# gssales/gaussian-splatting-reflection

Measured on AMD Instinct MI355X. Metric: train_step_views_per_s (fwd+bwd, 1e6 Gaussians @1080p, surfel rasterizer + reflection path), higher is better.
Workload: dtype f32

## Files before the change

### gaussian-splatting-reflection_amd/_gsr.py

```python
import ctypes
import os

import torch

_HERE = os.path.dirname(os.path.abspath(__file__))
LIB_PATH = os.environ.get("GSR_LIB") or os.path.join(_HERE, "libgsr_hip.so")

c_void_p, c_int, c_float, c_size_t, c_uint32, c_char_p = (ctypes.c_void_p, ctypes.c_int, ctypes.c_float, ctypes.c_size_t,
                                                         ctypes.c_uint32, ctypes.c_char_p)
ALLOC_FN = ctypes.CFUNCTYPE(c_void_p, c_void_p, c_int, c_size_t)

GSR_BUF_GEOM, GSR_BUF_BINNING, GSR_BUF_IMAGE = 0, 1, 2
GSR_PRESENT_CLAMP, GSR_PRESENT_QUANT8 = 1, 2
GSR_VIEW_HALF, GSR_VIEW_SOBEL, GSR_VIEW_COLORMAP = 1, 2, 4


class GsrError(RuntimeError):
    pass


class GatherGroup(ctypes.Structure):
    _fields_ = [("src_offset", ctypes.c_uint64), ("dst_offset", ctypes.c_uint64), ("width", c_uint32)]


# ... 136 lines not shown
def compiled_binding():
    want = os.environ.get("GSR_BINDING", "auto")
    if want == "ctypes":
        return None
    import importlib.util
    path = os.path.join(_HERE, "_gsr_C.so")
    if not os.path.exists(path):
        if want == "pybind":
            raise ImportError(f"GSR_BINDING=pybind but {path} is not built: run `python {os.path.join(_HERE, 'csrc', 'build.py')} --binding`")
        return None
    try:
        spec = importlib.util.spec_from_file_location("_gsr_C", path)
        mod = importlib.util.module_from_spec(spec)
        spec.loader.exec_module(mod)
        return mod
    except Exception:
        if want == "pybind":
            raise
        return None


PYBIND = compiled_binding()

EXPORTED = ["gsr_last_error", "gsr_version", "gsr_surfel_forward", "gsr_surfel_backward", "gsr_surfel_backward_accum", "gsr_surfel_backward_ex",
            "gsr_surfel_forward_refl", "gsr_surfel_forward_eval", "gsr_deferred_reflection_backward_keys", "gsr_deferred_reflection_forward_keys",
            "gsr_deferred_reflection_backward_accum", "gsr_deferred_reflection_backward_ex", "gsr_deferred_reflection_forward_ex", "gsr_side_join", "gsr_normal_world_forward", "gsr_normal_world_backward", "gsr_gauss_forward", "gsr_gauss_backward", "gsr_gauss_backward_accum",
            "gsr_mark_visible", "gsr_debug_fetch", "gsr_cubemap_forward", "gsr_cubemap_backward", "gsr_deferred_reflection_forward",
            "gsr_deferred_reflection_scratch_floats", "gsr_deferred_reflection_backward", "gsr_ssim_l1_scratch_floats", "gsr_ssim_l1_forward", "gsr_ssim_l1_backward", "gsr_normal_loss_scratch_floats", "gsr_normal_loss_forward", "gsr_normal_loss_backward", "gsr_adam_step", "gsr_adam_step_range", "gsr_densification_stats", "gsr_gather_rows", "gsr_split_children", "gsr_surface_forward", "gsr_surface_backward", "gsr_profile_enable",
            "gsr_profile_collect", "gsr_set_option", "gsr_knn_scratch_bytes", "gsr_knn_mean_dist",
            "gsr_image_metrics_scratch_floats", "gsr_image_metrics", "gsr_normal_mae_scratch_floats", "gsr_normal_mae",
            "gsr_present_view_scratch_floats", "gsr_present_view"]

STAGES = ["preprocess", "scan_readback", "emit_keys", "sort", "tile_ranges", "render_fwd", "render_bwd", "preprocess_bwd", "refl_fwd",
          "refl_bwd", "cubemap_fwd", "cubemap_bwd", "loss_fwd", "loss_bwd", "adam", "surface_fwd", "surface_bwd", "refl_bwd_tail"]


def set_option(name, value):
    check(lib.gsr_set_option(name.encode(), int(value)), f"gsr_set_option({name})")


_side_held = {}


def side_hold(*tensors):
    for t in tensors:
        if t is None:
            continue
        dev = t.device.index if t.device.index is not None else torch.cuda.current_device()
        _side_held.setdefault(dev, []).append((t, torch.cuda.current_stream(t.device).cuda_stream))


def side_join(device=None):
    dev = torch.device("cuda", torch.cuda.current_device()) if device is None else torch.device(device)
    if dev.index is None:
        dev = torch.device("cuda", torch.cuda.current_device())
    held = _side_held.pop(dev.index, [])
    with torch.cuda.device(dev):
        cur = torch.cuda.current_stream(dev).cuda_stream
        check(lib.gsr_side_join(cur), "gsr_side_join")
        for s in {s for _, s in held if s != cur}:
            check(lib.gsr_side_join(s), "gsr_side_join")
    del held


def profile_enable(on=True):
    lib.gsr_profile_enable(1 if on else 0)

# ... 107 lines not shown
```

### gaussian-splatting-reflection_amd/csrc/gsr_common.hip

```cpp
#include "gsr_internal.hpp"
#include <cstdarg>
#include <string>
#include <initializer_list>
#include <vector>
#include <mutex>
#include "gsr_sort.hpp"
#include <rocprim/device/device_scan.hpp>
#include <rocprim/iterator/counting_iterator.hpp>
#include <rocprim/iterator/transform_iterator.hpp>

namespace gsr {

static thread_local char g_err[512] = "";
void set_error(const char* fmt, ...) {
	va_list ap;
	va_start(ap, fmt);
	vsnprintf(g_err, sizeof(g_err), fmt, ap);
	va_end(ap);
}


struct ProfRec {
	int stage;
	hipEvent_t e0, e1;
// ... 5 lines not shown

StageTimer::StageTimer(int stage_, hipStream_t stream_) : stage(stage_), stream(stream_), rec(nullptr) {
	if (!g_prof_on) return;
	std::lock_guard<std::mutex> lk(g_prof_mu);
	ProfRec* r = nullptr;
	if (!g_prof_free.empty()) {
		r = g_prof_free.back();
		g_prof_free.pop_back();
	} else {
		r = new ProfRec();
		if (hipEventCreate(&r->e0) != hipSuccess || hipEventCreate(&r->e1) != hipSuccess) { delete r; return; }
	}
	r->stage = stage;
	(void)hipEventRecord(r->e0, stream);
	rec = r;
}
StageTimer::~StageTimer() {
	if (!rec) return;
	ProfRec* r = (ProfRec*)rec;
	(void)hipEventRecord(r->e1, stream);
	std::lock_guard<std::mutex> lk(g_prof_mu);
	g_prof_recs.push_back(r);
}

static int g_opt_cull = 1;
int option_cull() { return g_opt_cull; }
static int g_opt_dev = 0;
int option_dev() { return g_opt_dev; }
static int g_opt_emit_items = 0;
static int g_opt_mailbox = 1;
static int option_mailbox() { return g_opt_mailbox; }
static int g_opt_sort_driver = GSR_ONESWEEP_DRIVER;
int option_sort_driver() { return GSR_ONESWEEP_DRIVER && g_opt_sort_driver; }

uint32_t higher_msb(uint32_t n) {
	uint32_t msb = sizeof(n) * 4;
	uint32_t step = msb;
	while (step > 1) {
		step /= 2;
		if (n >> msb) msb += step;
		else msb -= step;
	}
	if (n >> msb) msb++;
	return msb;
}

using SortConfig = rocprim::radix_sort_config<rocprim::default_config, rocprim::default_config, rocprim::default_config, 65536>;
#ifndef DEPTH_SORT_BS
#define DEPTH_SORT_BS 1024
#endif
#ifndef DEPTH_SORT_IPT
#define DEPTH_SORT_IPT 4
#endif
#define DEPTH_SORT_SHAPE DEPTH_SORT_BS, DEPTH_SORT_IPT, 8
#define DEPTH_KEY_BITS 31u
#define DEPTH_KEY_PLACES 4u
#ifndef TILE_SORT_IPT
#define TILE_SORT_IPT 16
#endif
#ifndef TILE_SORT_BITS
#define TILE_SORT_BITS 8
#endif
#ifndef TILE_SORT_BS
#define TILE_SORT_BS 1024
#endif
#define TILE_SORT_SHAPE TILE_SORT_BS, TILE_SORT_IPT, TILE_SORT_BITS
// ... 506 lines not shown
	out[3 * idx + 0] = b & 1;
	out[3 * idx + 1] = (b >> 1) & 1;
	out[3 * idx + 2] = (b >> 2) & 1;
}
struct RecPick { int n; int pos[9]; };
__global__ void __launch_bounds__(256) pick_rec_kernel(int P, const float* __restrict__ rec, int stride, RecPick pick, float* __restrict__ out) {
	const int i = blockIdx.x * 256 + threadIdx.x;
	if (i >= P * pick.n) return;
	const int idx = i / pick.n, k = i % pick.n;
	out[i] = rec[(size_t)idx * stride + pick.pos[k]];
}
__global__ void __launch_bounds__(256) gather_rec_kernel(int P, const float* __restrict__ rec, int stride, int first, int nf,
                                                         float* __restrict__ out) {
	const int i = blockIdx.x * 256 + threadIdx.x;
	if (i >= P * nf) return;
	const int idx = i / nf, k = i % nf;
	out[i] = rec[(size_t)idx * stride + first + k];
}

}

using namespace gsr;

extern "C" const char* gsr_last_error(void) { return g_err; }
extern "C" int gsr_version(void) { return GSR_ABI_VERSION; }


extern "C" int gsr_set_option(const char* name, int value) {
	if (std::string(name) == "cull") { g_opt_cull = value ? 1 : 0; return 0; }
	if (std::string(name) == "dev") { g_opt_dev = value; return 0; }
	if (std::string(name) == "emit_items") { g_opt_emit_items = (value == 1 || value == 2) ? value : 0; return 0; }
	if (std::string(name) == "mailbox") { g_opt_mailbox = value ? 1 : 0; return 0; }
	if (std::string(name) == "sort_driver") { g_opt_sort_driver = value ? 1 : 0; return 0; }
	set_error("gsr_set_option: unknown option '%s'", name);
	return GSR_E_INVALID;
}
extern "C" int gsr_profile_enable(int on) {
	std::lock_guard<std::mutex> lk(g_prof_mu);
	for (ProfRec* r : g_prof_recs) g_prof_free.push_back(r);
	g_prof_recs.clear();
	g_prof_on = on != 0;
	return 0;
}
extern "C" int gsr_profile_collect(float* ms_out, int* launches_out) {
	std::lock_guard<std::mutex> lk(g_prof_mu);
	for (int i = 0; i < GSR_STAGE_COUNT; i++) { if (ms_out) ms_out[i] = 0.f; if (launches_out) launches_out[i] = 0; }
	for (ProfRec* r : g_prof_recs) {
		float ms = 0.f;
		if (hipEventSynchronize(r->e1) == hipSuccess && hipEventElapsedTime(&ms, r->e0, r->e1) == hipSuccess) {
			if (ms_out) ms_out[r->stage] += ms;
			if (launches_out) launches_out[r->stage] += 1;
		}
		g_prof_free.push_back(r);
	}
	g_prof_recs.clear();
	return 0;
}

extern "C" int gsr_mark_visible(int P, const float* means3D, const float* viewmatrix, const float* projmatrix, uint8_t* present,
                                void* stream_) {
	(void)projmatrix;
	hipStream_t stream = (hipStream_t)stream_;
	if (P < 0 || (P > 0 && (!means3D || !viewmatrix || !present))) { set_error("gsr_mark_visible: invalid argument"); return GSR_E_INVALID; }
	if (P == 0) return 0;
	mark_visible_kernel<<<(P + 255) / 256, 256, 0, stream>>>(P, means3D, viewmatrix, present);
	GSR_LAUNCH_CHECK(0, stream);
	return 0;
}

extern "C" int gsr_debug_fetch(int variant, const char* name, int P, int R, int width, int height, const void* geom_buffer,
                               const void* binning_buffer, const void* image_buffer, void* dst, void* stream_) {
	hipStream_t stream = (hipStream_t)stream_;
	const int tiles_x = (width + 15) / 16, tiles_y = (height + 15) / 16;
	const size_t HW = (size_t)width * height, tiles = (size_t)tiles_x * tiles_y;
	const WorkspaceLayout& layout = variant == 0 ? SURFEL_LAYOUT : GAUSS_LAYOUT;
	const int stride = layout.rec_f4 * 4;
	GeomState g = carve_geom((void*)geom_buffer, P, layout, nullptr);
	ImageState im = carve_image((void*)image_buffer, HW, tiles, layout, nullptr);
	BinningState b = carve_binning((void*)binning_buffer, R, tiles, 0, nullptr);
	auto d2d = [&](const void* src, size_t bytes) -> int {
		if (bytes == 0) return 0;
		GSR_HIP_CHECK(hipMemcpyAsync(dst, src, bytes, hipMemcpyDeviceToDevice, stream));
		return 0;
	};
	auto gather = [&](int first, int nf) -> int {
		if (P == 0) return 0;
		gather_rec_kernel<<<(P * nf + 255) / 256, 256, 0, stream>>>(P, (const float*)g.rec, stride, first, nf, (float*)dst);
		GSR_LAUNCH_CHECK(0, stream);
		return 0;
	};
	std::string n(name);
	if (n == "depths") return d2d(g.depths, (size_t)P * 4);
	if (n == "means2D") return gather(0, 2);

	if (n == "tiles_touched") return d2d(g.tiles_touched, (size_t)P * 4);
	if (n == "cull") return d2d(g.bbox, (size_t)P * 32);
	if (n == "point_offsets") {
		if (P == 0) return 0;
		size_t tmp = (size_t)(static_cast<char*>(g.depth_sort_temp) - static_cast<char*>(g.scan_temp));
		GSR_HIP_CHECK(rocprim::inclusive_scan(g.scan_temp, tmp, g.tiles_touched, g.point_offsets, (size_t)P, rocprim::plus<uint32_t>(), stream, false));
		return d2d(g.point_offsets, (size_t)P * 4);
	}
	if (n == "clamped") {
		if (P == 0) return 0;
		widen_clamped_kernel<<<(P + 255) / 256, 256, 0, stream>>>(P, g.clamped, (uint8_t*)dst);
		GSR_LAUNCH_CHECK(0, stream);
		return 0;
	}
	auto pick = [&](std::initializer_list<int> pos) -> int {
		if (P == 0) return 0;
		RecPick pk;
		pk.n = (int)pos.size();
		int i = 0;
		for (int v : pos) pk.pos[i++] = v;
		pick_rec_kernel<<<(P * pk.n + 255) / 256, 256, 0, stream>>>(P, (const float*)g.rec, stride, pk, (float*)dst);
		GSR_LAUNCH_CHECK(0, stream);
		return 0;
	};
	if (n == "rgb") return variant == 0 ? gather(16, 3) : gather(6, 3);
	if (n == "geom4") {
		return variant == 0 ? pick({12, 13, 14, 11}) : gather(2, 4);
	}
	if (n == "transMat" && variant == 0) return pick({2, 4, 6, 3, 5, 7, 8, 9, 10});
	if (n == "cov3D" && variant == 1) { set_error("gsr_debug_fetch: the 3D covariance is not kept by the forward (round 4: the backward recomputes it)"); return GSR_E_INVALID; }
	if (n == "point_list") return d2d(b.point_list, (size_t)R * 4);
	if (n == "keys") {
		if (R == 0) return 0;
		rebuild_keys_kernel<<<(R + 255) / 256, 256, 0, stream>>>(R, b.tile_keys, b.point_list, g.depths, (uint64_t*)dst);
// ... 10 lines not shown
```

### gaussian-splatting-reflection_amd/csrc/gsr_internal.hpp

```cpp
#pragma once
#include <cstring>
#include <cstdint>
#include <cstdio>
#include <hip/hip_runtime.h>
#include "../../include/gsr_hip.h"

#define GSR_TILE 16
#define GSR_TILE_PIX 256

namespace gsr {

void set_error(const char* fmt, ...);
#define GSR_HIP_CHECK(expr)                                                                       \
	do {                                                                                          \
		hipError_t _e = (expr);                                                                   \
		if (_e != hipSuccess) {                                                                   \
			gsr::set_error("%s failed: %s (%s:%d)", #expr, hipGetErrorString(_e), __FILE__, __LINE__); \
			return GSR_E_HIP;                                                                     \
		}                                                                                         \
	} while (0)
#define GSR_LAUNCH_CHECK(debug, stream)                                  \
	do {                                                                 \
		GSR_HIP_CHECK(hipGetLastError());                                \
		if (debug) GSR_HIP_CHECK(hipStreamSynchronize(stream));          \
// ... 103 lines not shown
};
static inline RasterCam make_cam(const float* view, const float* proj, const float* campos, int W, int H, float tan_fovx, float tan_fovy) {
	RasterCam c;
	c.view = view; c.proj = proj; c.campos = campos; c.W = W; c.H = H;
	c.tan_fovx = tan_fovx; c.tan_fovy = tan_fovy;
	c.focal_y = H / (2.0f * tan_fovy);
	c.focal_x = W / (2.0f * tan_fovx);
	return c;
}

struct BackwardWorkspace { GeomState geom; ImageState img; BinningState bin; int tiles_x, ntiles; };
static inline int backward_prologue(const char* entry, const char* func, const WorkspaceLayout& layout, int P, int M, int R, int width, int height,
                                    bool missing_pointer, const float* shs, const float* dL_dsh, const float* dL_drot, const float* also_aligned,
                                    const char* also_what, void* geom_buffer, void* binning_buffer, void* image_buffer, hipStream_t stream,
                                    BackwardWorkspace* w) {
	if (P < 0 || R < 0 || width <= 0 || height <= 0) { set_error("%s: invalid size", entry); return GSR_E_INVALID; }
	if (P == 0) return 0;
	if (missing_pointer) { set_error("%s: missing required pointer", entry); return GSR_E_INVALID; }
	if (shs && ((M * 3) & 3) == 0) GSR_REQUIRE_ALIGNED16_IN(func, shs, "shs (rows of a multiple of 16 bytes)");
	if (shs && ((M * 3) & 3) == 0) GSR_REQUIRE_ALIGNED16_IN(func, dL_dsh, "dL_dsh");
	GSR_REQUIRE_ALIGNED16_IN(func, dL_drot, "dL_drot");
	GSR_REQUIRE_ALIGNED16_IN(func, also_aligned, also_what);
	w->tiles_x = (width + 15) / 16;
	w->ntiles = w->tiles_x * ((height + 15) / 16);
	w->geom = carve_geom(geom_buffer, P, layout, nullptr);
	w->img = carve_image(image_buffer, (size_t)width * height, w->ntiles, layout, nullptr);
	w->bin = carve_binning(binning_buffer, R, w->ntiles, 0, nullptr);
	GSR_HIP_CHECK(hipMemsetAsync(w->geom.acc, 0, (size_t)P * layout.acc_floats * sizeof(float), stream));
	return 1;
}

int option_cull();
int option_dev();
size_t sort_temp_bytes(size_t R, int end_bit);
int run_tile_order(const ImageState& img, size_t tiles, hipStream_t stream);
uint32_t higher_msb(uint32_t n);

int run_binning(gsr_alloc_fn alloc, void* alloc_user, int P, int tiles_x, int tiles_y, const GeomState& geom,
                const ImageState& img, BinningState* out_binning, int prefiltered, int debug, hipStream_t stream, bool blend_masks = true);

int side_gate_wait(hipStream_t stream);
int refl_sort_keys_early(uint32_t L, int width, int height, float* scratch, size_t scratch_floats, const uint32_t* sort_keys, int async, bool gated,
                         hipStream_t stream);

}

#ifdef __HIPCC__
namespace gsr {

__device__ __forceinline__ int f2i(float v) { return (int)v; }

__device__ __forceinline__ void get_rect(float px, float py, int max_radius, int gx, int gy, uint32_t& x0, uint32_t& y0,
                                         uint32_t& x1, uint32_t& y1) {
	const float r = (float)max_radius;
	x0 = (uint32_t)min(gx, max(0, f2i((px - r) / 16.0f)));
	y0 = (uint32_t)min(gy, max(0, f2i((py - r) / 16.0f)));
	x1 = (uint32_t)min(gx, max(0, f2i((px + r + 15.0f) / 16.0f)));
	y1 = (uint32_t)min(gy, max(0, f2i((py + r + 15.0f) / 16.0f)));
}

#define GSR_DPP1(CTRL, i) "v_add_f32_dpp %" #i ", %" #i ", %" #i " " CTRL "\n\t"
#define GSR_DPP4(CTRL) GSR_DPP1(CTRL, 0) GSR_DPP1(CTRL, 1) GSR_DPP1(CTRL, 2) GSR_DPP1(CTRL, 3)
#define GSR_SHR1 "row_shr:1 row_mask:0xf bank_mask:0xf bound_ctrl:0"
#define GSR_SHR2 "row_shr:2 row_mask:0xf bank_mask:0xf bound_ctrl:0"
#define GSR_SHR4 "row_shr:4 row_mask:0xf bank_mask:0xf bound_ctrl:0"
#define GSR_SHR8 "row_shr:8 row_mask:0xf bank_mask:0xf bound_ctrl:0"
#define GSR_BC15 "row_bcast:15 row_mask:0xa bank_mask:0xf"
#define GSR_BC31 "row_bcast:31 row_mask:0xc bank_mask:0xf"
__device__ __forceinline__ void wave_sum4(float* v) {
	asm volatile("s_nop 1\n\t" GSR_DPP4(GSR_SHR1) GSR_DPP4(GSR_SHR2) GSR_DPP4(GSR_SHR4) GSR_DPP4(GSR_SHR8) GSR_DPP4(GSR_BC15) GSR_DPP4(GSR_BC31)
	             : "+v"(v[0]), "+v"(v[1]), "+v"(v[2]), "+v"(v[3]));
}

#define GSR_Q1(CTRL, i) "v_add_f32_dpp %" #i ", %" #i ", %" #i " " CTRL " row_mask:0xf bank_mask:0xf\n\t"
#define GSR_DPPB(CTRL, BANK, dst, src) "v_add_f32_dpp %" #dst ", %" #src ", %" #src " " CTRL " row_mask:0xf bank_mask:" BANK "\n\t"
#define GSR_L1(CTRL, d, a, b) GSR_DPPB(CTRL, "0x3", d, a) GSR_DPPB(CTRL, "0xc", d, b)
// ... 208 lines not shown
```

### gaussian-splatting-reflection_amd/csrc/gsr_surfel.hip

```cpp
#include <type_traits>
#include "gsr_internal.hpp"
#include "gsr_tile_walk.hpp"
#include "gsr_sort.hpp"
#include "gsr_math.hpp"
#include "gsr_refl.hpp"

namespace gsr {

#define SA_COLOR 0
#define SA_REFL 3
#define SA_NORMAL 4
#define SA_OPAC 7
#define SA_T 8
#define SA_MEAN2D 17

#define S_NEAR 0.2f
#define S_FAR 100.0f
#define S_FILTER_INV_SQ 2.0f

__device__ __forceinline__ M3 quat_to_rotmat(const float* __restrict__ q, float& w, float& x, float& y, float& z) {
#pragma clang fp contract(off)
	const float s = 1.0f / sqrtf(q[3] * q[3] + q[0] * q[0] + q[1] * q[1] + q[2] * q[2]);
	w = q[0] * s; x = q[1] * s; y = q[2] * s; z = q[3] * s;
	return m3_make(1.f - 2.f * (y * y + z * z), 2.f * (x * y + w * z), 2.f * (x * z - w * y), 2.f * (x * y - w * z),
// ... 44 lines not shown
	}
	const float* vm = cam.view;
	const float nx = R.m[2][0], ny = R.m[2][1], nz = R.m[2][2];
	normal = f3(vm[0] * nx + vm[4] * ny + vm[8] * nz, vm[1] * nx + vm[5] * ny + vm[9] * nz, vm[2] * nx + vm[6] * ny + vm[10] * nz);
}

__device__ __forceinline__ void surfel_cull_record(const M3& T, float cx, float cy, float opa, float4& c0, float4& c1) {
	c0 = make_float4(cx, cy, 0.f, 0.f);
	c1 = make_float4(0.f, cx, cy, -2.0f);
	if (!(opa >= 1.0f / 255.0f)) return;
	const float c2f = 2.0f * logf(255.0f * opa) * 1.05f + 0.1f;
	c1.w = 0.5f * c2f * 1.02f;
	const double ic2 = 1.0 / (double)c2f;
	const double a00 = T.m[0][0], a01 = T.m[0][1], a02 = T.m[0][2];
	const double a10 = T.m[1][0], a11 = T.m[1][1], a12 = T.m[1][2];
	const double a20 = T.m[2][0], a21 = T.m[2][1], a22 = T.m[2][2];
	const double sigma = a20 * a20 + a21 * a21 - a22 * a22 * ic2;
	if (!(sigma < -1e-6 * a22 * a22 * ic2)) return;
	const double sx = a00 * a20 + a01 * a21 - a02 * a22 * ic2, sy = a10 * a20 + a11 * a21 - a12 * a22 * ic2;
	const double Sxx = a00 * a00 + a01 * a01 - a02 * a02 * ic2, Sxy = a00 * a10 + a01 * a11 - a02 * a12 * ic2,
	             Syy = a10 * a10 + a11 * a11 - a12 * a12 * ic2;
	const double is = 1.0 / sigma;
	const double ex = sx * is, ey = sy * is;
	const double g = -is * 1.0404;
	const double Vxx = (Sxx - sx * sx * is) * g + 0.25, Vxy = (Sxy - sx * sy * is) * g, Vyy = (Syy - sy * sy * is) * g + 0.25;
	const double det = Vxx * Vyy - Vxy * Vxy;
	if (!(Vxx > 0.25) || !(Vyy > 0.25) || !(det > 0.0)) return;
	const float fa = (float)(Vyy / det), fb = (float)(-Vxy / det), fc = (float)(Vxx / det);
	if (!(fa > 0.f) || !(fc > 0.f) || !(fa * fc - fb * fb > 0.f) || !(fabsf((float)ex) < 1e7f) || !(fabsf((float)ey) < 1e7f)) return;
	c0 = make_float4((float)ex, (float)ey, fa, fb);
	c1.x = fc;
}

template <bool TRAIN>
__device__ __forceinline__ bool
surfel_preprocess_one(int idx, int D, int M, const float* __restrict__ means, const float* __restrict__ scales, float scale_modifier,
                      const float* __restrict__ rotations, const float* __restrict__ opacities, const float* __restrict__ shs,
                      const float* __restrict__ transMat_precomp, const float* __restrict__ colors_precomp, const float* __restrict__ refl,
                      const uint8_t* __restrict__ env_scope_mask, const RasterCam& cam, int* __restrict__ radii, const GeomState& g, int gx, int gy,
                      int prefiltered, float* __restrict__ gaussian_weights, float4* o) {
#pragma clang fp contract(off)
	radii[idx] = 0;
	if constexpr (TRAIN) gaussian_weights[idx] = 0.f;
	g.tiles_touched[idx] = 0;
	reinterpret_cast<uint2*>(g.rect)[idx] = make_uint2(0u, 0u);
	g.depths[idx] = __int_as_float(0x7f7fffff);
	const float mx = means[3 * idx], my = means[3 * idx + 1], mz = means[3 * idx + 2];
	const float* vm = cam.view;
	const float pvx = vm[0] * mx + vm[4] * my + vm[8] * mz + vm[12];
	const float pvy = vm[1] * mx + vm[5] * my + vm[9] * mz + vm[13];
	const float pvz = vm[2] * mx + vm[6] * my + vm[10] * mz + vm[14];
	if (pvz <= 0.2f) {
		if (prefiltered) g.flags[0] = 1;
		return false;
	}
	M3 T;
	F3 normal;
	if (transMat_precomp == nullptr) {
		compute_transmat(mx, my, mz, scales + 2 * idx, scale_modifier, rotations + 4 * idx, cam, T, normal);
	} else {
#pragma unroll
		for (int c = 0; c < 3; c++)
#pragma unroll
			for (int r = 0; r < 3; r++) T.m[c][r] = transMat_precomp[9 * idx + 3 * c + r];
		normal = f3(0.0f, 0.0f, 1.0f);
	}
	const float cosv = -((pvx * normal.x) + (pvy * normal.y) + (pvz * normal.z));
	if (cosv == 0) return false;
	const float multiplier = cosv > 0 ? 1.f : -1.f;
	normal = f3(multiplier * normal.x, multiplier * normal.y, multiplier * normal.z);
	const float cutoff = 3.0f;
	const float t0 = cutoff * cutoff, t1 = cutoff * cutoff, t2 = -1.0f;
	const float d = t0 * (T.m[2][0] * T.m[2][0]) + t1 * (T.m[2][1] * T.m[2][1]) + t2 * (T.m[2][2] * T.m[2][2]);
	if (d == 0.0f) return false;
	const float inv_d = 1 / d;
	const float f0 = inv_d * t0, f1 = inv_d * t1, f2 = inv_d * t2;
	const float pxi = f0 * (T.m[0][0] * T.m[2][0]) + f1 * (T.m[0][1] * T.m[2][1]) + f2 * (T.m[0][2] * T.m[2][2]);
	const float pyi = f0 * (T.m[1][0] * T.m[2][0]) + f1 * (T.m[1][1] * T.m[2][1]) + f2 * (T.m[1][2] * T.m[2][2]);
	const float h0x = pxi * pxi - (f0 * (T.m[0][0] * T.m[0][0]) + f1 * (T.m[0][1] * T.m[0][1]) + f2 * (T.m[0][2] * T.m[0][2]));
	const float h0y = pyi * pyi - (f0 * (T.m[1][0] * T.m[1][0]) + f1 * (T.m[1][1] * T.m[1][1]) + f2 * (T.m[1][2] * T.m[1][2]));
	const float ex = sqrtf(fmaxf(1e-4f, h0x)), ey = sqrtf(fmaxf(1e-4f, h0y));
	const float radius = ceilf(fmaxf(fmaxf(ex, ey), cutoff * (float)0.707106));
	uint32_t x0, y0, x1, y1;
	get_rect(pxi, pyi, f2i(radius), gx, gy, x0, y0, x1, y1);
	if ((x1 - x0) * (y1 - y0) == 0) return false;

	float cr, cg, cb;
	if (colors_precomp == nullptr) {
		const float dx = mx - cam.campos[0], dy = my - cam.campos[1], dz = mz - cam.campos[2];
		const float len = sqrtf(dx * dx + dy * dy + dz * dz);
		ShRow s;
		load_sh(shs, idx, M, (D + 1) * (D + 1), s);
		const F3 c = sh_eval(D, s, dx / len, dy / len, dz / len);
		if constexpr (TRAIN) g.clamped[idx] = (uint8_t)((c.x < 0 ? 1 : 0) | (c.y < 0 ? 2 : 0) | (c.z < 0 ? 4 : 0));
		cr = fmaxf(c.x, 0.0f); cg = fmaxf(c.y, 0.0f); cb = fmaxf(c.z, 0.0f);
	} else {
		cr = colors_precomp[3 * idx]; cg = colors_precomp[3 * idx + 1]; cb = colors_precomp[3 * idx + 2];
	}
	g.depths[idx] = pvz;
	radii[idx] = f2i(radius);
	g.rect[2 * idx] = x0 | (y0 << 16);
	g.rect[2 * idx + 1] = x1 | (y1 << 16);
	const float maskv = (env_scope_mask != nullptr && env_scope_mask[idx]) ? 1.0f : 0.0f;
	surfel_cull_record(T, pxi, pyi, opacities[idx], o[5], o[6]);
	float4* rec = o;
	rec[0] = make_float4(pxi, pyi, T.m[0][0], T.m[1][0]);
	rec[1] = make_float4(T.m[0][1], T.m[1][1], T.m[0][2], T.m[1][2]);
	rec[2] = make_float4(T.m[2][0], T.m[2][1], T.m[2][2], opacities[idx]);
	rec[3] = make_float4(normal.x, normal.y, normal.z, refl[idx]);
	rec[4] = make_float4(cr, cg, cb, maskv);
	g.tiles_touched[idx] = (y1 - y0) * (x1 - x0);
	return true;
}

#define S_OUT_F4 7
struct CubemapInterleave {
	const float* cubemap;
	float4* rgba;
	uint32_t ntex, LL;
};
template <bool TRAIN>
__global__ void __launch_bounds__(256)
surfel_preprocess_kernel(int P, int D, int M, const float* __restrict__ means, const float* __restrict__ scales, float scale_modifier,
                         const float* __restrict__ rotations, const float* __restrict__ opacities, const float* __restrict__ shs,
                         const float* __restrict__ transMat_precomp, const float* __restrict__ colors_precomp,
                         const float* __restrict__ refl, const uint8_t* __restrict__ env_scope_mask, RasterCam cam, int* __restrict__ radii,
                         GeomState g, int gx, int gy, int prefiltered, float* __restrict__ gaussian_weights, CubemapInterleave ci) {
	const int idx = blockIdx.x * 256 + threadIdx.x;
	for (uint32_t t = (uint32_t)idx; t < ci.ntex; t += gridDim.x * 256u) {
		const uint32_t f = t / ci.LL, r = t - f * ci.LL;
		const float* c = ci.cubemap + (size_t)f * 3 * ci.LL + r;
		ci.rgba[t] = make_float4(c[0], c[ci.LL], c[2 * (size_t)ci.LL], 0.f);
	}
	sort_clear_region(g.depth_sort_temp, g.depth_sort_clear, (size_t)idx, (size_t)gridDim.x * 256u);
	sort_clear_region(g.emit_state, g.emit_state_bytes, (size_t)idx, (size_t)gridDim.x * 256u);
	if (idx == 0) { g.flags[1] = 0; g.flags[2] = 0; g.flags[3] = 0; }
	__shared__ float4 s_out[4][S_REC_F4 * 65];
	const int lane = threadIdx.x & 63;
	float4* so = s_out[threadIdx.x >> 6];
	float4 o[S_OUT_F4];
#pragma unroll
	for (int k = 0; k < S_OUT_F4; k++) o[k] = make_float4(0.f, 0.f, 0.f, 0.f);
	bool live = false;
	if (idx < P)
		live = surfel_preprocess_one<TRAIN>(idx, D, M, means, scales, scale_modifier, rotations, opacities, shs, transMat_precomp, colors_precomp, refl,
		                             env_scope_mask, cam, radii, g, gx, gy, prefiltered, gaussian_weights, o);
	if (__ballot(live) == 0ull) return;
	const int g0 = idx - lane;
	const int ng = min(64, P - g0);
	wave_store_rows4<S_REC_F4, false>(so, o, g.rec + (size_t)g0 * S_REC_F4, S_REC_F4, 0, ng, lane);
	wave_store_rows4<2, false>(so, o + S_REC_F4, g.bbox + (size_t)g0 * 2, 2, 0, ng, lane);
}

typedef float v2f __attribute__((ext_vector_type(2)));
__device__ __forceinline__ v2f mk2(float a, float b) { v2f r; r.x = a; r.y = b; return r; }

struct SurfelRec : TileRec<S_REC_F4> {
	__device__ __forceinline__ v2f xy() const { return mk2(f[0].x, f[0].y); }
	__device__ __forceinline__ v2f TuvX() const { return mk2(f[0].z, f[0].w); }
	__device__ __forceinline__ v2f TuvY() const { return mk2(f[1].x, f[1].y); }
	__device__ __forceinline__ v2f TuvZ() const { return mk2(f[1].z, f[1].w); }
	__device__ __forceinline__ v2f Twxy() const { return mk2(f[2].x, f[2].y); }
	__device__ __forceinline__ float Twz() const { return f[2].z; }
	__device__ __forceinline__ float opac() const { return f[2].w; }
	__device__ __forceinline__ v2f nxy() const { return mk2(f[3].x, f[3].y); }
	__device__ __forceinline__ float nz() const { return f[3].z; }
	__device__ __forceinline__ float refl() const { return f[3].w; }
	__device__ __forceinline__ v2f rg() const { return mk2(f[4].x, f[4].y); }
	__device__ __forceinline__ float b() const { return f[4].z; }
	__device__ __forceinline__ float mask() const { return f[4].w; }
};

#ifndef GSR_BWD_WPE
#define GSR_BWD_WPE 4
#endif
#ifndef GSR_BWD_LIST
#define GSR_BWD_LIST 1
#endif
#ifndef GSR_BWD_UNROLL
// ... 793 lines not shown
	if (P == 0) {
		float* normal = TRAIN ? out_others + 2 * HW : out_normal_view;
		if (!normal) {
			normal = static_cast<float*>(alloc(alloc_user, GSR_BUF_IMAGE, HW * 3 * 4));
			if (!normal) { set_error("workspace allocation failed (%zu bytes)", HW * 3 * 4); return GSR_E_ALLOC; }
		}
		GSR_HIP_CHECK(hipMemsetAsync(out_color, 0, HW * 3 * 4, stream));
		if (TRAIN) {
			GSR_HIP_CHECK(hipMemsetAsync(out_others, 0, HW * 8 * 4, stream));
		} else {
			GSR_HIP_CHECK(hipMemsetAsync(out_alpha, 0, HW * 4, stream));
			GSR_HIP_CHECK(hipMemsetAsync(normal, 0, HW * 3 * 4, stream));
		}
		GSR_HIP_CHECK(hipMemsetAsync(out_refl_strength_map, 0, HW * 4, stream));
		if (refl && gsr_deferred_reflection_forward_keys(normal, out_color, out_refl_strength_map, refl->cam, refl->cubemap, refl->fail_value, refl->L,
		                                                 width, height, refl->out_final, refl->out_refl_color, refl->out_normal_world, refl->cubemap_rgba,
		                                                 refl->sort_keys, stream) < 0)
			return GSR_E_HIP;
	} else {
		const int tiles_x = (width + 15) / 16, tiles_y = (height + 15) / 16;
		const int ntiles = tiles_x * tiles_y;
		GeomState geom; ImageState img;
		if (const int rc = forward_workspace(alloc, alloc_user, TRAIN ? SURFEL_LAYOUT : SURFEL_LAYOUT.inference(), P, HW, ntiles, &geom, &img); rc < 0) return rc;

		if (prefiltered) GSR_HIP_CHECK(hipMemsetAsync(geom.flags, 0, 4 * sizeof(int), stream));
		const RasterCam cam = make_cam(viewmatrix, projmatrix, cam_pos, width, height, tan_fovx, tan_fovy);
		CubemapInterleave ci{nullptr, nullptr, 0u, 1u};
		SurfelReflFwd rf{};
		if (refl) {
			ci = CubemapInterleave{refl->cubemap, reinterpret_cast<float4*>(refl->cubemap_rgba), 6u * refl->L * refl->L, refl->L * refl->L};
			rf = SurfelReflFwd{refl->cam, refl->cubemap, reinterpret_cast<const float4*>(refl->cubemap_rgba), refl->fail_value, (int)refl->L, 6u * refl->L * refl->L,
			                   refl->out_final, refl->out_refl_color, refl->out_normal_world, refl->sort_keys};
		}
	{ StageTimer st_(GSR_STAGE_PREPROCESS, stream); 	surfel_preprocess_kernel<TRAIN><<<(P + 255) / 256, 256, 0, stream>>>(P, D, M, means3D, scales, scale_modifier, rotations, opacities, shs,
		                                                                     transMat_precomp, colors_precomp, refl_strengths, env_scope_mask, cam, radii, geom,
		                                                                     tiles_x, tiles_y, prefiltered, gaussian_weights, ci); }
		GSR_LAUNCH_CHECK(debug, stream);

		BinningState bin;
		R = run_binning(alloc, alloc_user, P, tiles_x, tiles_y, geom, img, &bin, prefiltered, debug, stream, TRAIN);
		if (R < 0) return R;

	{ StageTimer st_(GSR_STAGE_RENDER_FWD, stream);
		const int nunits = (int)xcd_grid((uint32_t)ntiles * 4u);
		const auto args = [&] { if constexpr (TRAIN) return rf; else return SurfelEvalFwd{rf, out_alpha, out_normal_view}; }();
		auto render = refl ? surfel_render_fwd_wave_kernel<true, TRAIN> : surfel_render_fwd_wave_kernel<false, TRAIN>;
		render<<<nunits, 64, 0, stream>>>(img.ranges, img.tile_order, bin.point_list, width, height, tiles_x, ntiles, geom.rec, geom.bbox, option_cull(),
		                                  background, TRAIN ? img.final_T : nullptr, TRAIN ? img.n_contrib : nullptr, out_color, out_others,
		                                  out_refl_strength_map, gaussian_weights, bin.blend_mask, bin.mask_stride, args); }
		GSR_LAUNCH_CHECK(debug, stream);
	}
	if (const int rc = TRAIN ? early_key_sort(refl, width, height, R, stream) : 0; rc < 0) return rc;
	return R;
}

extern "C" int gsr_surfel_forward_refl(gsr_alloc_fn alloc, void* alloc_user, int P, int D, int M, const float* background, int width, int height,
                                  const float* means3D, const uint8_t* env_scope_mask, const float* shs, const float* colors_precomp,
                                  const float* refl_strengths, const float* opacities, const float* scales, float scale_modifier,
                                  const float* rotations, const float* transMat_precomp, const float* viewmatrix, const float* projmatrix,
                                  const float* cam_pos, float tan_fovx, float tan_fovy, int prefiltered, float* out_color, float* out_others,
                                  float* out_refl_strength_map, int* radii, float* gaussian_weights, const gsr_refl_forward* refl, int debug,
                                  void* stream_) {
	if (!alloc || P < 0 || width <= 0 || height <= 0 || !background || !out_color || !out_others || !out_refl_strength_map) {
		set_error("gsr_surfel_forward: invalid argument");
		return GSR_E_INVALID;
	}
	if (P > 0 && !gaussian_weights) { set_error("gsr_surfel_forward: missing required input pointer"); return GSR_E_INVALID; }
	if (const int rc = check_refl_descriptor("gsr_surfel_forward_refl", refl); rc < 0) return rc;
	if (const int rc = check_surfel_inputs("gsr_surfel_forward", P, D, M, means3D, shs, colors_precomp, refl_strengths, opacities, scales, rotations,
	                                       transMat_precomp, viewmatrix, projmatrix, cam_pos, radii); rc < 0) return rc;
	return surfel_forward<true>(alloc, alloc_user, P, D, M, background, width, height, means3D, env_scope_mask, shs, colors_precomp, refl_strengths,
	                            opacities, scales, scale_modifier, rotations, transMat_precomp, viewmatrix, projmatrix, cam_pos, tan_fovx, tan_fovy,
	                            prefiltered, out_color, out_others, nullptr, nullptr, out_refl_strength_map, radii, gaussian_weights, refl, debug,
	                            (hipStream_t)stream_);
// ... 101 lines not shown
```

### include/gsr_hip.h

```cpp
#ifndef GSR_HIP_H_
#define GSR_HIP_H_

#include <stddef.h>
#include <stdint.h>

#ifdef __cplusplus
extern "C" {
#endif

#define GSR_BUF_GEOM 0
#define GSR_BUF_BINNING 1
#define GSR_BUF_IMAGE 2

#define GSR_E_INVALID (-1)
#define GSR_E_HIP (-2)
#define GSR_E_ALLOC (-3)
#define GSR_E_PREFILTERED (-4)
#define GSR_E_NONRGB (-5)

typedef void* (*gsr_alloc_fn)(void* user, int which, size_t bytes);

const char* gsr_last_error(void);
#define GSR_ABI_VERSION 102
int gsr_version(void);
// ... 201 lines not shown
                            float* scratch, void* stream);
int gsr_normal_loss_backward(const float* rend_normal, const float* surf_normal, const float* mask, int H, int W,
                             const float* g_sum, float* g_rend_normal, float* g_surf_normal, void* stream);
typedef struct {
	uint64_t begin, end;
	float lr, lr2;
	uint32_t period, split;
} gsr_adam_segment;
int gsr_adam_step(float* param, const float* grad, float* exp_avg, float* exp_avg_sq, uint64_t n,
                  const gsr_adam_segment* segments, int num_segments, float beta1, float beta2, float eps, int step,
                  void* stream);
int gsr_adam_step_range(float* param, const float* grad, float* exp_avg, float* exp_avg_sq, uint64_t n,
                        const gsr_adam_segment* segments, int num_segments, float beta1, float beta2, float eps, int step,
                        uint64_t range_begin, uint64_t range_end, void* stream);

#define GSR_STAGE_PREPROCESS 0
#define GSR_STAGE_SCAN 1
#define GSR_STAGE_EMIT_KEYS 2
#define GSR_STAGE_SORT 3
#define GSR_STAGE_RANGES 4
#define GSR_STAGE_RENDER_FWD 5
#define GSR_STAGE_RENDER_BWD 6
#define GSR_STAGE_PREPROCESS_BWD 7
#define GSR_STAGE_REFL_FWD 8
#define GSR_STAGE_REFL_BWD 9
#define GSR_STAGE_CUBEMAP_FWD 10
#define GSR_STAGE_CUBEMAP_BWD 11
#define GSR_STAGE_LOSS_FWD 12
#define GSR_STAGE_LOSS_BWD 13
#define GSR_STAGE_ADAM 14
#define GSR_STAGE_SURFACE_FWD 15
#define GSR_STAGE_SURFACE_BWD 16
#define GSR_STAGE_REFL_BWD_TAIL 17
#define GSR_STAGE_COUNT 18
int gsr_set_option(const char* name, int value);
int gsr_profile_enable(int on);
int gsr_profile_collect(float* ms_out , int* launches_out );

#ifdef __cplusplus
}
#endif
#endif
```

Measured before the change: 541.9.

## Split surfel preprocess into binning-key kernel and helper-stream record kernel

Factors the depth/rect/tiles-touched computation out of the surfel preprocess into a lightweight bin-keys kernel. In split mode the full record preprocess (SH colours, records) runs on a low-priority helper stream that overlaps binning and sort, and is joined before rendering. Split mode is off by default; the default path instead uses a fused kernel that runs bin-keys and then the record preprocess in one launch. That fused path recomputes the view position, transform matrix and AABB for each Gaussian, which adds arithmetic.

After: 352.6. 0.651x the previous value.

```diff
diff --git a/gaussian-splatting-reflection_amd/_gsr.py b/gaussian-splatting-reflection_amd/_gsr.py
--- a/gaussian-splatting-reflection_amd/_gsr.py
+++ b/gaussian-splatting-reflection_amd/_gsr.py
@@ -192,7 +192,7 @@
             "gsr_present_view_scratch_floats", "gsr_present_view"]
 
 STAGES = ["preprocess", "scan_readback", "emit_keys", "sort", "tile_ranges", "render_fwd", "render_bwd", "preprocess_bwd", "refl_fwd",
-          "refl_bwd", "cubemap_fwd", "cubemap_bwd", "loss_fwd", "loss_bwd", "adam", "surface_fwd", "surface_bwd", "refl_bwd_tail"]
+          "refl_bwd", "cubemap_fwd", "cubemap_bwd", "loss_fwd", "loss_bwd", "adam", "surface_fwd", "surface_bwd", "refl_bwd_tail", "bin_keys", "helper_join"]
 
 
 def set_option(name, value):
diff --git a/gaussian-splatting-reflection_amd/csrc/gsr_common.hip b/gaussian-splatting-reflection_amd/csrc/gsr_common.hip
--- a/gaussian-splatting-reflection_amd/csrc/gsr_common.hip
+++ b/gaussian-splatting-reflection_amd/csrc/gsr_common.hip
@@ -61,6 +61,86 @@
 static int option_mailbox() { return g_opt_mailbox; }
 static int g_opt_sort_driver = GSR_ONESWEEP_DRIVER;
 int option_sort_driver() { return GSR_ONESWEEP_DRIVER && g_opt_sort_driver; }
+
+#ifndef SPLIT_PREPROCESS_FROM
+#define SPLIT_PREPROCESS_FROM 0
+#endif
+static int g_opt_split = -1;
+int split_preprocess_mode(int P, int prefiltered, int debug) {
+	if (g_opt_split == 0) return 1;
+	if (prefiltered || debug) return 0;
+	return (g_opt_split == 1 || (SPLIT_PREPROCESS_FROM > 0 && P >= SPLIT_PREPROCESS_FROM)) ? 2 : 0;
+}
+
+namespace {
+struct Helper {
+	hipStream_t stream = nullptr;
+	hipEvent_t fork = nullptr, done = nullptr;
+};
+std::mutex g_helper_mu;
+Helper g_helper[64];
+Helper* helper_slot() {
+	int dev = 0;
+	if (hipGetDevice(&dev) != hipSuccess || dev < 0 || dev >= 64) return nullptr;
+	Helper& h = g_helper[dev];
+	if (!h.stream) {
+		int least = 0, greatest = 0;
+		(void)hipDeviceGetStreamPriorityRange(&least, &greatest);
+		if (hipStreamCreateWithPriority(&h.stream, hipStreamNonBlocking, least) != hipSuccess) { h.stream = nullptr; return nullptr; }
+		if (hipEventCreateWithFlags(&h.fork, hipEventDisableTiming) != hipSuccess || hipEventCreateWithFlags(&h.done, hipEventDisableTiming) != hipSuccess) {
+			(void)hipStreamDestroy(h.stream);
+			h.stream = nullptr;
+		}
+	}
+	return h.stream ? &h : nullptr;
+}
+}
+
+int HelperFork::fork() {
+	g_helper_mu.lock();
+	locked_ = true;
+	Helper* h = helper_slot();
+	if (!h) { set_error("the forward's helper stream could not be created"); g_helper_mu.unlock(); locked_ = false; return GSR_E_HIP; }
+	side_ = h;
+	hipError_t e = hipEventRecord(h->fork, caller_);
+	if (e == hipSuccess) e = hipStreamWaitEvent(h->stream, h->fork, 0);
+	if (e != hipSuccess) {
+		set_error("fork to the helper stream failed: %s", hipGetErrorString(e));
+		g_helper_mu.unlock();
+		locked_ = false;
+		return GSR_E_HIP;
+	}
+	helper_ = h->stream;
+	pending_ = true;
+	return 0;
+}
+int HelperFork::done() {
+	Helper* h = static_cast<Helper*>(side_);
+	hipError_t e = hipEventRecord(h->done, h->stream);
+	if (e != hipSuccess) {
+		(void)hipStreamSynchronize(h->stream);
+		pending_ = false;
+	}
+	g_helper_mu.unlock();
+	locked_ = false;
+	if (e != hipSuccess) { set_error("hipEventRecord on the helper stream failed: %s", hipGetErrorString(e)); return GSR_E_HIP; }
+	return 0;
+}
+int HelperFork::join() {
+	if (!pending_) return 0;
+	pending_ = false;
+	Helper* h = static_cast<Helper*>(side_);
+	if (locked_) {
+		(void)hipStreamSynchronize(h->stream);
+		g_helper_mu.unlock();
+		locked_ = false;
+		return 0;
+	}
+	std::lock_guard<std::mutex> lk(g_helper_mu);
+	if (hipStreamWaitEvent(caller_, h->done, 0) != hipSuccess) GSR_HIP_CHECK(hipStreamSynchronize(h->stream));
+	return 0;
+}
+HelperFork::~HelperFork() { (void)join(); }
 
 uint32_t higher_msb(uint32_t n) {
 	uint32_t msb = sizeof(n) * 4;
@@ -633,6 +713,11 @@
 	if (std::string(name) == "emit_items") { g_opt_emit_items = (value == 1 || value == 2) ? value : 0; return 0; }
 	if (std::string(name) == "mailbox") { g_opt_mailbox = value ? 1 : 0; return 0; }
 	if (std::string(name) == "sort_driver") { g_opt_sort_driver = value ? 1 : 0; return 0; }
+	if (std::string(name) == "split_preprocess") {
+		if (value < -1 || value > 1) { set_error("gsr_set_option: split_preprocess takes -1, 0 or 1, not %d", value); return GSR_E_INVALID; }
+		g_opt_split = value;
+		return 0;
+	}
 	set_error("gsr_set_option: unknown option '%s'", name);
 	return GSR_E_INVALID;
 }
@@ -695,6 +780,7 @@
 	if (n == "means2D") return gather(0, 2);
 
 	if (n == "tiles_touched") return d2d(g.tiles_touched, (size_t)P * 4);
+	if (n == "rect") return d2d(g.rect, (size_t)P * 8);
 	if (n == "cull") return d2d(g.bbox, (size_t)P * 32);
 	if (n == "point_offsets") {
 		if (P == 0) return 0;
diff --git a/gaussian-splatting-reflection_amd/csrc/gsr_internal.hpp b/gaussian-splatting-reflection_amd/csrc/gsr_internal.hpp
--- a/gaussian-splatting-reflection_amd/csrc/gsr_internal.hpp
+++ b/gaussian-splatting-reflection_amd/csrc/gsr_internal.hpp
@@ -159,6 +159,7 @@
 
 int option_cull();
 int option_dev();
+int split_preprocess_mode(int P, int prefiltered, int debug);
 size_t sort_temp_bytes(size_t R, int end_bit);
 int run_tile_order(const ImageState& img, size_t tiles, hipStream_t stream);
 uint32_t higher_msb(uint32_t n);
@@ -169,6 +170,22 @@
 int side_gate_wait(hipStream_t stream);
 int refl_sort_keys_early(uint32_t L, int width, int height, float* scratch, size_t scratch_floats, const uint32_t* sort_keys, int async, bool gated,
                          hipStream_t stream);
+
+class HelperFork {
+public:
+	explicit HelperFork(hipStream_t caller) : caller_(caller) {}
+	~HelperFork();
+	HelperFork(const HelperFork&) = delete;
+	HelperFork& operator=(const HelperFork&) = delete;
+	int fork();
+	hipStream_t stream() const { return helper_; }
+	int done();
+	int join();
+private:
+	hipStream_t caller_, helper_ = nullptr;
+	void* side_ = nullptr;
+	bool locked_ = false, pending_ = false;
+};
 
 }
 
diff --git a/gaussian-splatting-reflection_amd/csrc/gsr_surfel.hip b/gaussian-splatting-reflection_amd/csrc/gsr_surfel.hip
--- a/gaussian-splatting-reflection_amd/csrc/gsr_surfel.hip
+++ b/gaussian-splatting-reflection_amd/csrc/gsr_surfel.hip
@@ -100,58 +100,110 @@
 	c1.x = fc;
 }
 
+
+__device__ __forceinline__ F3 surfel_view_pos(const RasterCam& cam, float mx, float my, float mz) {
+#pragma clang fp contract(off)
+	const float* vm = cam.view;
+	return f3(vm[0] * mx + vm[4] * my + vm[8] * mz + vm[12], vm[1] * mx + vm[5] * my + vm[9] * mz + vm[13], vm[2] * mx + vm[6] * my + vm[10] * mz + vm[14]);
+}
+__device__ __forceinline__ bool surfel_transmat(int idx, float mx, float my, float mz, const F3& pv, const float* __restrict__ scales, float scale_modifier,
+                                                const float* __restrict__ rotations, const float* __restrict__ transMat_precomp, const RasterCam& cam,
+                                                M3& T, F3& normal) {
+#pragma clang fp contract(off)
+	if (transMat_precomp == nullptr) {
+		compute_transmat(mx, my, mz, scales + 2 * idx, scale_modifier, rotations + 4 * idx, cam, T, normal);
+	} else {
+#pragma unroll
+		for (int c = 0; c < 3; c++)
+#pragma unroll
+			for (int r = 0; r < 3; r++) T.m[c][r] = transMat_precomp[9 * idx + 3 * c + r];
+		normal = f3(0.0f, 0.0f, 1.0f);
+	}
+	const float cosv = -((pv.x * normal.x) + (pv.y * normal.y) + (pv.z * normal.z));
+	if (cosv == 0) return false;
+	const float multiplier = cosv > 0 ? 1.f : -1.f;
+	normal = f3(multiplier * normal.x, multiplier * normal.y, multiplier * normal.z);
+	return true;
+}
+#define S_CUTOFF 3.0f
+__device__ __forceinline__ bool surfel_aabb(const M3& T, float& pxi, float& pyi, float& ex, float& ey) {
+#pragma clang fp contract(off)
+	const float cutoff = S_CUTOFF;
+	const float t0 = cutoff * cutoff, t1 = cutoff * cutoff, t2 = -1.0f;
+	const float d = t0 * (T.m[2][0] * T.m[2][0]) + t1 * (T.m[2][1] * T.m[2][1]) + t2 * (T.m[2][2] * T.m[2][2]);
+	if (d == 0.0f) return false;
+	const float inv_d = 1 / d;
+	const float f0 = inv_d * t0, f1 = inv_d * t1, f2 = inv_d * t2;
+	pxi = f0 * (T.m[0][0] * T.m[2][0]) + f1 * (T.m[0][1] * T.m[2][1]) + f2 * (T.m[0][2] * T.m[2][2]);
+	pyi = f0 * (T.m[1][0] * T.m[2][0]) + f1 * (T.m[1][1] * T.m[2][1]) + f2 * (T.m[1][2] * T.m[2][2]);
+	const float h0x = pxi * pxi - (f0 * (T.m[0][0] * T.m[0][0]) + f1 * (T.m[0][1] * T.m[0][1]) + f2 * (T.m[0][2] * T.m[0][2]));
+	const float h0y = pyi * pyi - (f0 * (T.m[1][0] * T.m[1][0]) + f1 * (T.m[1][1] * T.m[1][1]) + f2 * (T.m[1][2] * T.m[1][2]));
+	ex = sqrtf(fmaxf(1e-4f, h0x));
+	ey = sqrtf(fmaxf(1e-4f, h0y));
+	return true;
+}
+
+__device__ __forceinline__ void surfel_bin_clears(const GeomState& g, size_t thread, size_t threads) {
+	sort_clear_region(g.depth_sort_temp, g.depth_sort_clear, thread, threads);
+	sort_clear_region(g.emit_state, g.emit_state_bytes, thread, threads);
+	if (thread == 0) { g.flags[1] = 0; g.flags[2] = 0; g.flags[3] = 0; }
+}
+__device__ __forceinline__ void surfel_bin_keys_one(int idx, const float* __restrict__ means, const float* __restrict__ scales, float scale_modifier,
+                                                    const float* __restrict__ rotations, const float* __restrict__ transMat_precomp, const RasterCam& cam,
+                                                    int* __restrict__ radii, const GeomState& g, int gx, int gy, int prefiltered) {
+#pragma clang fp contract(off)
+	int radius = 0;
+	uint32_t touched = 0;
+	uint2 rect = make_uint2(0u, 0u);
+	float depth = __int_as_float(0x7f7fffff);
+	const float mx = means[3 * idx], my = means[3 * idx + 1], mz = means[3 * idx + 2];
+	const F3 pv = surfel_view_pos(cam, mx, my, mz);
+	if (pv.z <= 0.2f) {
+		if (prefiltered) g.flags[0] = 1;
+	} else {
+		M3 T;
+		F3 normal;
+		float pxi, pyi, ex, ey;
+		if (surfel_transmat(idx, mx, my, mz, pv, scales, scale_modifier, rotations, transMat_precomp, cam, T, normal) && surfel_aabb(T, pxi, pyi, ex, ey)) {
+			const float r = ceilf(fmaxf(fmaxf(ex, ey), S_CUTOFF * (float)0.707106));
+			uint32_t x0, y0, x1, y1;
+			get_rect(pxi, pyi, f2i(r), gx, gy, x0, y0, x1, y1);
+			if ((x1 - x0) * (y1 - y0) != 0) {
+				depth = pv.z;
+				radius = f2i(r);
+				rect = make_uint2(x0 | (y0 << 16), x1 | (y1 << 16));
+				touched = (y1 - y0) * (x1 - x0);
+			}
+		}
+	}
+	radii[idx] = radius;
+	g.tiles_touched[idx] = touched;
+	reinterpret_cast<uint2*>(g.rect)[idx] = rect;
+	g.depths[idx] = depth;
+}
+__global__ void __launch_bounds__(256)
+surfel_bin_keys_kernel(int P, const float* __restrict__ means, const float* __restrict__ scales, float scale_modifier, const float* __restrict__ rotations,
+                       const float* __restrict__ transMat_precomp, RasterCam cam, int* __restrict__ radii, GeomState g, int gx, int gy, int prefiltered) {
+	const int idx = blockIdx.x * 256 + threadIdx.x;
+	surfel_bin_clears(g, (size_t)idx, (size_t)gridDim.x * 256u);
+	if (idx < P) surfel_bin_keys_one(idx, means, scales, scale_modifier, rotations, transMat_precomp, cam, radii, g, gx, gy, prefiltered);
+}
+
 template <bool TRAIN>
 __device__ __forceinline__ bool
 surfel_preprocess_one(int idx, int D, int M, const float* __restrict__ means, const float* __restrict__ scales, float scale_modifier,
                       const float* __restrict__ rotations, const float* __restrict__ opacities, const float* __restrict__ shs,
                       const float* __restrict__ transMat_precomp, const float* __restrict__ colors_precomp, const float* __restrict__ refl,
-                      const uint8_t* __restrict__ env_scope_mask, const RasterCam& cam, int* __restrict__ radii, const GeomState& g, int gx, int gy,
-                      int prefiltered, float* __restrict__ gaussian_weights, float4* o) {
+                      const uint8_t* __restrict__ env_scope_mask, const RasterCam& cam, const GeomState& g, float* __restrict__ gaussian_weights, float4* o) {
 #pragma clang fp contract(off)
-	radii[idx] = 0;
 	if constexpr (TRAIN) gaussian_weights[idx] = 0.f;
-	g.tiles_touched[idx] = 0;
-	reinterpret_cast<uint2*>(g.rect)[idx] = make_uint2(0u, 0u);
-	g.depths[idx] = __int_as_float(0x7f7fffff);
+	if (g.tiles_touched[idx] == 0) return false;
 	const float mx = means[3 * idx], my = means[3 * idx + 1], mz = means[3 * idx + 2];
-	const float* vm = cam.view;
-	const float pvx = vm[0] * mx + vm[4] * my + vm[8] * mz + vm[12];
-	const float pvy = vm[1] * mx + vm[5] * my + vm[9] * mz + vm[13];
-	const float pvz = vm[2] * mx + vm[6] * my + vm[10] * mz + vm[14];
-	if (pvz <= 0.2f) {
-		if (prefiltered) g.flags[0] = 1;
-		return false;
-	}
 	M3 T;
 	F3 normal;
-	if (transMat_precomp == nullptr) {
-		compute_transmat(mx, my, mz, scales + 2 * idx, scale_modifier, rotations + 4 * idx, cam, T, normal);
-	} else {
-#pragma unroll
-		for (int c = 0; c < 3; c++)
-#pragma unroll
-			for (int r = 0; r < 3; r++) T.m[c][r] = transMat_precomp[9 * idx + 3 * c + r];
-		normal = f3(0.0f, 0.0f, 1.0f);
-	}
-	const float cosv = -((pvx * normal.x) + (pvy * normal.y) + (pvz * normal.z));
-	if (cosv == 0) return false;
-	const float multiplier = cosv > 0 ? 1.f : -1.f;
-	normal = f3(multiplier * normal.x, multiplier * normal.y, multiplier * normal.z);
-	const float cutoff = 3.0f;
-	const float t0 = cutoff * cutoff, t1 = cutoff * cutoff, t2 = -1.0f;
-	const float d = t0 * (T.m[2][0] * T.m[2][0]) + t1 * (T.m[2][1] * T.m[2][1]) + t2 * (T.m[2][2] * T.m[2][2]);
-	if (d == 0.0f) return false;
-	const float inv_d = 1 / d;
-	const float f0 = inv_d * t0, f1 = inv_d * t1, f2 = inv_d * t2;
-	const float pxi = f0 * (T.m[0][0] * T.m[2][0]) + f1 * (T.m[0][1] * T.m[2][1]) + f2 * (T.m[0][2] * T.m[2][2]);
-	const float pyi = f0 * (T.m[1][0] * T.m[2][0]) + f1 * (T.m[1][1] * T.m[2][1]) + f2 * (T.m[1][2] * T.m[2][2]);
-	const float h0x = pxi * pxi - (f0 * (T.m[0][0] * T.m[0][0]) + f1 * (T.m[0][1] * T.m[0][1]) + f2 * (T.m[0][2] * T.m[0][2]));
-	const float h0y = pyi * pyi - (f0 * (T.m[1][0] * T.m[1][0]) + f1 * (T.m[1][1] * T.m[1][1]) + f2 * (T.m[1][2] * T.m[1][2]));
-	const float ex = sqrtf(fmaxf(1e-4f, h0x)), ey = sqrtf(fmaxf(1e-4f, h0y));
-	const float radius = ceilf(fmaxf(fmaxf(ex, ey), cutoff * (float)0.707106));
-	uint32_t x0, y0, x1, y1;
-	get_rect(pxi, pyi, f2i(radius), gx, gy, x0, y0, x1, y1);
-	if ((x1 - x0) * (y1 - y0) == 0) return false;
+	float pxi, pyi, ex, ey;
+	(void)surfel_transmat(idx, mx, my, mz, surfel_view_pos(cam, mx, my, mz), scales, scale_modifier, rotations, transMat_precomp, cam, T, normal);
+	(void)surfel_aabb(T, pxi, pyi, ex, ey);
 
 	float cr, cg, cb;
 	if (colors_precomp == nullptr) {
@@ -165,10 +217,6 @@
 	} else {
 		cr = colors_precomp[3 * idx]; cg = colors_precomp[3 * idx + 1]; cb = colors_precomp[3 * idx + 2];
 	}
-	g.depths[idx] = pvz;
-	radii[idx] = f2i(radius);
-	g.rect[2 * idx] = x0 | (y0 << 16);
-	g.rect[2 * idx + 1] = x1 | (y1 << 16);
 	const float maskv = (env_scope_mask != nullptr && env_scope_mask[idx]) ? 1.0f : 0.0f;
 	surfel_cull_record(T, pxi, pyi, opacities[idx], o[5], o[6]);
 	float4* rec = o;
@@ -177,7 +225,6 @@
 	rec[2] = make_float4(T.m[2][0], T.m[2][1], T.m[2][2], opacities[idx]);
 	rec[3] = make_float4(normal.x, normal.y, normal.z, refl[idx]);
 	rec[4] = make_float4(cr, cg, cb, maskv);
-	g.tiles_touched[idx] = (y1 - y0) * (x1 - x0);
 	return true;
 }
 
@@ -187,7 +234,7 @@
 	float4* rgba;
 	uint32_t ntex, LL;
 };
-template <bool TRAIN>
+template <bool TRAIN, bool FUSED>
 __global__ void __launch_bounds__(256)
 surfel_preprocess_kernel(int P, int D, int M, const float* __restrict__ means, const float* __restrict__ scales, float scale_modifier,
                          const float* __restrict__ rotations, const float* __restrict__ opacities, const float* __restrict__ shs,
@@ -195,14 +242,15 @@
                          const float* __restrict__ refl, const uint8_t* __restrict__ env_scope_mask, RasterCam cam, int* __restrict__ radii,
                          GeomState g, int gx, int gy, int prefiltered, float* __restrict__ gaussian_weights, CubemapInterleave ci) {
 	const int idx = blockIdx.x * 256 + threadIdx.x;
+	if constexpr (FUSED) {
+		surfel_bin_clears(g, (size_t)idx, (size_t)gridDim.x * 256u);
+		if (idx < P) surfel_bin_keys_one(idx, means, scales, scale_modifier, rotations, transMat_precomp, cam, radii, g, gx, gy, prefiltered);
+	}
 	for (uint32_t t = (uint32_t)idx; t < ci.ntex; t += gridDim.x * 256u) {
 		const uint32_t f = t / ci.LL, r = t - f * ci.LL;
 		const float* c = ci.cubemap + (size_t)f * 3 * ci.LL + r;
 		ci.rgba[t] = make_float4(c[0], c[ci.LL], c[2 * (size_t)ci.LL], 0.f);
 	}
-	sort_clear_region(g.depth_sort_temp, g.depth_sort_clear, (size_t)idx, (size_t)gridDim.x * 256u);
-	sort_clear_region(g.emit_state, g.emit_state_bytes, (size_t)idx, (size_t)gridDim.x * 256u);
-	if (idx == 0) { g.flags[1] = 0; g.flags[2] = 0; g.flags[3] = 0; }
 	__shared__ float4 s_out[4][S_REC_F4 * 65];
 	const int lane = threadIdx.x & 63;
 	float4* so = s_out[threadIdx.x >> 6];
@@ -212,7 +260,7 @@
 	bool live = false;
 	if (idx < P)
 		live = surfel_preprocess_one<TRAIN>(idx, D, M, means, scales, scale_modifier, rotations, opacities, shs, transMat_precomp, colors_precomp, refl,
-		                             env_scope_mask, cam, radii, g, gx, gy, prefiltered, gaussian_weights, o);
+		                                    env_scope_mask, cam, g, gaussian_weights, o);
 	if (__ballot(live) == 0ull) return;
 	const int g0 = idx - lane;
 	const int ng = min(64, P - g0);
@@ -1072,14 +1120,39 @@
 			rf = SurfelReflFwd{refl->cam, refl->cubemap, reinterpret_cast<const float4*>(refl->cubemap_rgba), refl->fail_value, (int)refl->L, 6u * refl->L * refl->L,
 			                   refl->out_final, refl->out_refl_color, refl->out_normal_world, refl->sort_keys};
 		}
-	{ StageTimer st_(GSR_STAGE_PREPROCESS, stream); 	surfel_preprocess_kernel<TRAIN><<<(P + 255) / 256, 256, 0, stream>>>(P, D, M, means3D, scales, scale_modifier, rotations, opacities, shs,
-		                                                                     transMat_precomp, colors_precomp, refl_strengths, env_scope_mask, cam, radii, geom,
-		                                                                     tiles_x, tiles_y, prefiltered, gaussian_weights, ci); }
+		const int mode = split_preprocess_mode(P, prefiltered, debug);
+		const bool split = mode == 2;
+		if (mode != 0) {
+			StageTimer st_(GSR_STAGE_BIN_KEYS, stream);
+			surfel_bin_keys_kernel<<<(P + 255) / 256, 256, 0, stream>>>(P, means3D, scales, scale_modifier, rotations, transMat_precomp, cam, radii, geom, tiles_x,
+			                                                           tiles_y, prefiltered);
+		}
 		GSR_LAUNCH_CHECK(debug, stream);
+		HelperFork helper(stream);
+		if (split) {
+			if (const int rc = helper.fork(); rc < 0) return rc;
+		}
+		const hipStream_t rec_stream = split ? helper.stream() : stream;
+		{
+			StageTimer st_(GSR_STAGE_PREPROCESS, rec_stream);
+			auto kern = mode == 0 ? surfel_preprocess_kernel<TRAIN, true> : surfel_preprocess_kernel<TRAIN, false>;
+			kern<<<(P + 255) / 256, 256, 0, rec_stream>>>(P, D, M, means3D, scales, scale_modifier, rotations, opacities, shs, transMat_precomp, colors_precomp,
+			                                              refl_strengths, env_scope_mask, cam, radii, geom, tiles_x, tiles_y, prefiltered, gaussian_weights, ci);
+		}
+		const hipError_t launched = hipGetLastError();
+		if (split) {
+			if (const int rc = helper.done(); rc < 0) return rc;
+		}
+		GSR_HIP_CHECK(launched);
+		if (debug) GSR_HIP_CHECK(hipStreamSynchronize(stream));
 
 		BinningState bin;
 		R = run_binning(alloc, alloc_user, P, tiles_x, tiles_y, geom, img, &bin, prefiltered, debug, stream, TRAIN);
 		if (R < 0) return R;
+		if (split) {
+			StageTimer st_(GSR_STAGE_HELPER_JOIN, stream);
+			if (const int rc = helper.join(); rc < 0) return rc;
+		}
 
 	{ StageTimer st_(GSR_STAGE_RENDER_FWD, stream);
 		const int nunits = (int)xcd_grid((uint32_t)ntiles * 4u);
diff --git a/include/gsr_hip.h b/include/gsr_hip.h
--- a/include/gsr_hip.h
+++ b/include/gsr_hip.h
@@ -257,7 +257,9 @@
 #define GSR_STAGE_SURFACE_FWD 15
 #define GSR_STAGE_SURFACE_BWD 16
 #define GSR_STAGE_REFL_BWD_TAIL 17
-#define GSR_STAGE_COUNT 18
+#define GSR_STAGE_BIN_KEYS 18
+#define GSR_STAGE_HELPER_JOIN 19
+#define GSR_STAGE_COUNT 20
 int gsr_set_option(const char* name, int value);
 int gsr_profile_enable(int on);
 int gsr_profile_collect(float* ms_out , int* launches_out );
```
